# localdevices/pyorc

Measured on AMD Instinct MI355X. Metric: PIV frame-pairs/sec, 1080p 32x32@50% overlap (Mvectors/sec in config), higher is better.
Workload: dtype f32; 1 GPU; synthetic 1080x1920 uint8 particle stack, 1000 frame-pairs per GPU, 32x32 windows @ overlap 16 (BASELINE.json configs[1]); frame_dtype=u8, windows_per_pair=7854, parallelism=single GPU

## Files before the change

pyorc_amd/csrc/fft_debug.hip:

```cpp
#include "piv_fft_impl.h"

namespace lspiv {

template <bool INV, int FORM> __device__ __forceinline__ void fft_form(float (&r)[16], float (&i)[16]) { fft16<INV, false, FORM == 2>(r, i); }
template <bool INV, int FORM> __device__ __forceinline__ void fft_form(float (&r)[32], float (&i)[32]) { fft32<INV, false, FORM == 2>(r, i); }
template <bool INV, int FORM> __device__ __forceinline__ void fft_form(float (&r)[64], float (&i)[64]) { fft64<INV, false, FORM == 2>(r, i); }

template <int N, bool INV, int FORM = 0>
__global__ void fft_debug_kernel(const float* in, float* out, int count) {
  const int t = blockIdx.x * blockDim.x + threadIdx.x;
  if (t >= count) return;
  float r[N], i[N];
#pragma unroll
  for (int j = 0; j < N; ++j) { r[j] = in[(size_t)t * 2 * N + 2 * j]; i[j] = in[(size_t)t * 2 * N + 2 * j + 1]; }
  if constexpr (FORM == 0) fft_n<INV>(r, i); else fft_form<INV, FORM>(r, i);
#pragma unroll
  for (int j = 0; j < N; ++j) { out[(size_t)t * 2 * N + 2 * j] = r[j]; out[(size_t)t * 2 * N + 2 * j + 1] = i[j]; }
}

template <int N, int FORM = 0>
static hipError_t launch_one(bool inverse, const float* in, float* out, int count, hipStream_t s) {
  const dim3 grid((count + 63) / 64), block(64);
  if (inverse) hipLaunchKernelGGL((fft_debug_kernel<N, true, FORM>), grid, block, 0, s, in, out, count);
  else hipLaunchKernelGGL((fft_debug_kernel<N, false, FORM>), grid, block, 0, s, in, out, count);
  return hipGetLastError();
}

hipError_t launch_fft_debug(int n, bool inverse, const float* in, float* out, int count, hipStream_t s) {
  switch (n) {
    case 8: return launch_one<8>(inverse, in, out, count, s);
    case 16: return launch_one<16>(inverse, in, out, count, s);
    case 32: return launch_one<32>(inverse, in, out, count, s);
    case 64: return launch_one<64>(inverse, in, out, count, s);
#define LSPIV_PFA_CASE(m) case m: return launch_one<m>(inverse, in, out, count, s);
    LSPIV_PFA_SIZES(LSPIV_PFA_CASE)
#undef LSPIV_PFA_CASE
    default: return hipErrorInvalidValue;
  }
}

hipError_t launch_fft_debug_form(int n, int form, bool inverse, const float* in, float* out, int count, hipStream_t s) {
  if (form == 0) return launch_fft_debug(n, inverse, in, out, count, s);
  if (form != 1 && form != 2) return hipErrorInvalidValue;
  switch (n) {
    case 16: return form == 1 ? launch_one<16, 1>(inverse, in, out, count, s) : launch_one<16, 2>(inverse, in, out, count, s);
    case 32: return form == 1 ? launch_one<32, 1>(inverse, in, out, count, s) : launch_one<32, 2>(inverse, in, out, count, s);
    case 64: return form == 1 ? launch_one<64, 1>(inverse, in, out, count, s) : launch_one<64, 2>(inverse, in, out, count, s);
    default: return hipErrorInvalidValue;
  }
}

}
```

pyorc_amd/csrc/fft_regs.h:

```cpp
#pragma once
#include <hip/hip_runtime.h>

namespace lspiv {

static constexpr float kCos64[64] = {
    1.0f, 0.9951847195625305f, 0.9807852506637573f, 0.9569403529167175f,
    0.9238795042037964f, 0.8819212913513184f, 0.8314695954322815f, 0.7730104327201843f,
    0.7071067690849304f, 0.6343932747840881f, 0.5555702447891235f, 0.4713967442512512f,
    0.3826834261417389f, 0.290284663438797f, 0.19509032368659973f, 0.0980171412229538f,
    0.0f, -0.0980171412229538f, -0.19509032368659973f, -0.290284663438797f,
    -0.3826834261417389f, -0.4713967442512512f, -0.5555702447891235f, -0.6343932747840881f,
    -0.7071067690849304f, -0.7730104327201843f, -0.8314695954322815f, -0.8819212913513184f,
    -0.9238795042037964f, -0.9569403529167175f, -0.9807852506637573f, -0.9951847195625305f,
    -1.0f, -0.9951847195625305f, -0.9807852506637573f, -0.9569403529167175f,
    -0.9238795042037964f, -0.8819212913513184f, -0.8314695954322815f, -0.7730104327201843f,
    -0.7071067690849304f, -0.6343932747840881f, -0.5555702447891235f, -0.4713967442512512f,
    -0.3826834261417389f, -0.290284663438797f, -0.19509032368659973f, -0.0980171412229538f,
    0.0f, 0.0980171412229538f, 0.19509032368659973f, 0.290284663438797f,
    0.3826834261417389f, 0.4713967442512512f, 0.5555702447891235f, 0.6343932747840881f,
    0.7071067690849304f, 0.7730104327201843f, 0.8314695954322815f, 0.8819212913513184f,
    0.9238795042037964f, 0.9569403529167175f, 0.9807852506637573f, 0.9951847195625305f};

__host__ __device__ constexpr float cos64(int m) { return kCos64[m & 63]; }
__host__ __device__ constexpr float sin64(int m) { return kCos64[(m - 16) & 63]; }

constexpr float kSqrtHalf = 0.70710678118654757f;

template <bool INV, int M>
__device__ __forceinline__ void twiddle64(float& xr, float& xi) {
  constexpr int m = M & 63;
  if constexpr (m == 0) {
    return;
  } else if constexpr (m == 16) {
    float t = xr;
    if constexpr (!INV) { xr = xi; xi = -t; } else { xr = -xi; xi = t; }
  } else if constexpr (m == 32) {
    xr = -xr; xi = -xi;
  } else if constexpr (m == 48) {
    float t = xr;
    if constexpr (!INV) { xr = -xi; xi = t; } else { xr = xi; xi = -t; }
  } else {
    constexpr float c = cos64(m);
    constexpr float s = INV ? sin64(m) : -sin64(m);
    float tr = xr * c - xi * s;
    float ti = xr * s + xi * c;
    xr = tr; xi = ti;
  }
}

template <bool CLAMP>
__device__ __forceinline__ float out01(float x) { return CLAMP ? __builtin_amdgcn_fmed3f(x, 0.0f, 1.0f) : x; }

template <bool INV, bool CLAMP>
__device__ __forceinline__ void bfly4_tail(float ar, float ai, float br, float bi, float cr, float ci, float dr, float di,
                                           float& r0, float& i0, float& r1, float& i1,
                                           float& r2, float& i2, float& r3, float& i3) {
  r0 = out01<CLAMP>(ar + cr); i0 = out01<CLAMP>(ai + ci);
  r2 = out01<CLAMP>(ar - cr); i2 = out01<CLAMP>(ai - ci);
  if constexpr (!INV) {
    r1 = out01<CLAMP>(br + di); i1 = out01<CLAMP>(bi - dr);
    r3 = out01<CLAMP>(br - di); i3 = out01<CLAMP>(bi + dr);
  } else {
    r1 = out01<CLAMP>(br - di); i1 = out01<CLAMP>(bi + dr);
    r3 = out01<CLAMP>(br + di); i3 = out01<CLAMP>(bi - dr);
  }
}

template <bool INV, bool CLAMP = false>
__device__ __forceinline__ void bfly4(float& r0, float& i0, float& r1, float& i1,
                                      float& r2, float& i2, float& r3, float& i3) {
  float ar = r0 + r2, ai = i0 + i2;
  float br = r0 - r2, bi = i0 - i2;
  float cr = r1 + r3, ci = i1 + i3;
  float dr = r1 - r3, di = i1 - i3;
  bfly4_tail<INV, CLAMP>(ar, ai, br, bi, cr, ci, dr, di, r0, i0, r1, i1, r2, i2, r3, i3);
}

template <bool INV, bool CLAMP>
__device__ __forceinline__ void bfly8_tail(float (&r)[8], float (&i)[8]) {
  {
    float tr = r[3], ti = i[3];
    if constexpr (!INV) { r[3] = (tr + ti) * kSqrtHalf; i[3] = (ti - tr) * kSqrtHalf; }
    else                { r[3] = (tr - ti) * kSqrtHalf; i[3] = (ti + tr) * kSqrtHalf; }
    tr = r[5]; ti = i[5];
    if constexpr (!INV) { r[5] = ti; i[5] = -tr; } else { r[5] = -ti; i[5] = tr; }
    tr = r[7]; ti = i[7];
    if constexpr (!INV) { r[7] = (ti - tr) * kSqrtHalf; i[7] = -(tr + ti) * kSqrtHalf; }
    else                { r[7] = -(tr + ti) * kSqrtHalf; i[7] = (tr - ti) * kSqrtHalf; }
  }
  float er[4] = {r[0], r[2], r[4], r[6]}, ei[4] = {i[0], i[2], i[4], i[6]};
  float orr[4] = {r[1], r[3], r[5], r[7]}, oi[4] = {i[1], i[3], i[5], i[7]};
#pragma unroll
  for (int k = 0; k < 4; ++k) {
    r[k] = out01<CLAMP>(er[k] + orr[k]);     i[k] = out01<CLAMP>(ei[k] + oi[k]);
    r[k + 4] = out01<CLAMP>(er[k] - orr[k]); i[k + 4] = out01<CLAMP>(ei[k] - oi[k]);
  }
}

template <bool INV, bool CLAMP = false>
__device__ __forceinline__ void bfly8(float (&r)[8], float (&i)[8]) {
  bfly4<INV>(r[0], i[0], r[2], i[2], r[4], i[4], r[6], i[6]);
  bfly4<INV>(r[1], i[1], r[3], i[3], r[5], i[5], r[7], i[7]);
  bfly8_tail<INV, CLAMP>(r, i);
}

template <bool INV, int N2, int K1, int STEP>
struct TwiddleRow {
  template <int n2>
  static __device__ __forceinline__ void apply(float (&r)[8], float (&i)[8]) {
    if constexpr (n2 < N2) {
      twiddle64<INV, STEP * n2 * K1>(r[n2], i[n2]);
      apply<n2 + 1>(r, i);
    }
  }
};

#ifdef LSPIV_FFT_FOLD
constexpr bool kFftFold16 = LSPIV_FFT_FOLD, kFftFold32 = LSPIV_FFT_FOLD, kFftFold64 = LSPIV_FFT_FOLD, kFftFoldWalk32 = LSPIV_FFT_FOLD;
#else
constexpr bool kFftFold16 = true, kFftFold32 = false, kFftFold64 = false, kFftFoldWalk32 = true;
#endif
template <int N> constexpr bool kFftFoldLen = N == 16 ? kFftFold16 : N == 32 ? kFftFold32 : N == 64 ? kFftFold64 : false;
template <int N> constexpr bool kFftFoldWalk = N == 32 ? kFftFoldWalk32 : kFftFoldLen<N>;

template <bool INV, int M>
struct FoldTw {
  static constexpr int m = M & 63;
  static constexpr bool triv = (m % 16) == 0;
  static constexpr double c = cos64(m), s = INV ? sin64(m) : -sin64(m);
  static constexpr bool sform = (s < 0 ? -s : s) > (c < 0 ? -c : c);
  static constexpr float t = triv ? 0.0f : (float)(sform ? c / s : s / c);
  static constexpr float kr = triv ? 1.0f : (float)(sform ? -s : c);
  static constexpr float ki = triv ? 1.0f : (float)(sform ? s : c);
};

template <bool INV, int M>
__device__ __forceinline__ void fold_u(float& vr, float& vi) {
  using T = FoldTw<INV, M>;
  if constexpr (T::triv) {
    twiddle64<INV, M>(vr, vi);
  } else if constexpr (!T::sform) {
    const float ur = fmaf(vi, -T::t, vr), ui = fmaf(vr, T::t, vi);
    vr = ur; vi = ui;
  } else {
    const float ur = fmaf(vr, -T::t, vi), ui = fmaf(vi, T::t, vr);
    vr = ur; vi = ui;
  }
}

template <bool TRIVX, bool TRIVY>
__device__ __forceinline__ void fold_pair(float x, float kx, float y, float ky, float& sum, float& dif) {
  if constexpr (TRIVX && TRIVY) {
    sum = x + y; dif = x - y;
  } else if constexpr (TRIVY) {
    const float p = kx * x;
    sum = p + y; dif = p - y;
  } else {
    const float p = TRIVX ? x : kx * x;
    sum = fmaf(y, ky, p); dif = fmaf(y, -ky, p);
  }
}

template <bool INV, bool CLAMP, int E0, int E1, int E2, int E3>
__device__ __forceinline__ void bfly4_fold(float& r0, float& i0, float& r1, float& i1,
                                           float& r2, float& i2, float& r3, float& i3) {
  using T0 = FoldTw<INV, E0>; using T1 = FoldTw<INV, E1>; using T2 = FoldTw<INV, E2>; using T3 = FoldTw<INV, E3>;
  fold_u<INV, E0>(r0, i0); fold_u<INV, E1>(r1, i1); fold_u<INV, E2>(r2, i2); fold_u<INV, E3>(r3, i3);
  float ar, ai, br, bi, cr, ci, dr, di;
  fold_pair<T0::triv, T2::triv>(r0, T0::kr, r2, T2::kr, ar, br);
  fold_pair<T0::triv, T2::triv>(i0, T0::ki, i2, T2::ki, ai, bi);
  fold_pair<T1::triv, T3::triv>(r1, T1::kr, r3, T3::kr, cr, dr);
  fold_pair<T1::triv, T3::triv>(i1, T1::ki, i3, T3::ki, ci, di);
  bfly4_tail<INV, CLAMP>(ar, ai, br, bi, cr, ci, dr, di, r0, i0, r1, i1, r2, i2, r3, i3);
}

template <bool INV, bool CLAMP, bool FOLD, int K1, int STEP>
__device__ __forceinline__ void twiddled_bfly8(float (&r)[8], float (&i)[8]) {
  if constexpr (FOLD) {
    constexpr int E = STEP * K1;
    bfly4_fold<INV, false, 0, 2 * E, 4 * E, 6 * E>(r[0], i[0], r[2], i[2], r[4], i[4], r[6], i[6]);
    bfly4_fold<INV, false, E, 3 * E, 5 * E, 7 * E>(r[1], i[1], r[3], i[3], r[5], i[5], r[7], i[7]);
    bfly8_tail<INV, CLAMP>(r, i);
  } else {
    TwiddleRow<INV, 8, K1, STEP>::template apply<1>(r, i);
    bfly8<INV, CLAMP>(r, i);
  }
}

template <bool INV, bool CLAMP, int K1>
__device__ __forceinline__ void fft16_row_fold(const float (&xr)[16], const float (&xi)[16], float (&yr)[16], float (&yi)[16]) {
  float r0 = xr[4 * K1], i0 = xi[4 * K1], r1 = xr[4 * K1 + 1], i1 = xi[4 * K1 + 1];
  float r2 = xr[4 * K1 + 2], i2 = xi[4 * K1 + 2], r3 = xr[4 * K1 + 3], i3 = xi[4 * K1 + 3];
  bfly4_fold<INV, CLAMP, 0, 4 * K1, 8 * K1, 12 * K1>(r0, i0, r1, i1, r2, i2, r3, i3);
  yr[K1] = r0; yi[K1] = i0; yr[K1 + 4] = r1; yi[K1 + 4] = i1; yr[K1 + 8] = r2; yi[K1 + 8] = i2; yr[K1 + 12] = r3; yi[K1 + 12] = i3;
}

template <bool INV, bool CLAMP = false, bool FOLD = kFftFold16>
__device__ __forceinline__ void fft16(float (&xr)[16], float (&xi)[16]) {
#pragma unroll
  for (int n2 = 0; n2 < 4; ++n2)
    bfly4<INV>(xr[n2], xi[n2], xr[4 + n2], xi[4 + n2], xr[8 + n2], xi[8 + n2], xr[12 + n2], xi[12 + n2]);
  if constexpr (FOLD) {
    float yr[16], yi[16];
    fft16_row_fold<INV, CLAMP, 0>(xr, xi, yr, yi); fft16_row_fold<INV, CLAMP, 1>(xr, xi, yr, yi);
    fft16_row_fold<INV, CLAMP, 2>(xr, xi, yr, yi); fft16_row_fold<INV, CLAMP, 3>(xr, xi, yr, yi);
#pragma unroll
    for (int k = 0; k < 16; ++k) { xr[k] = yr[k]; xi[k] = yi[k]; }
    return;
  }
  twiddle64<INV, 4 * 1 * 1>(xr[4 + 1], xi[4 + 1]);  twiddle64<INV, 4 * 2 * 1>(xr[4 + 2], xi[4 + 2]);  twiddle64<INV, 4 * 3 * 1>(xr[4 + 3], xi[4 + 3]);
  twiddle64<INV, 4 * 1 * 2>(xr[8 + 1], xi[8 + 1]);  twiddle64<INV, 4 * 2 * 2>(xr[8 + 2], xi[8 + 2]);  twiddle64<INV, 4 * 3 * 2>(xr[8 + 3], xi[8 + 3]);
  twiddle64<INV, 4 * 1 * 3>(xr[12 + 1], xi[12 + 1]); twiddle64<INV, 4 * 2 * 3>(xr[12 + 2], xi[12 + 2]); twiddle64<INV, 4 * 3 * 3>(xr[12 + 3], xi[12 + 3]);
  float yr[16], yi[16];
#pragma unroll
  for (int k1 = 0; k1 < 4; ++k1) {
    float r0 = xr[4 * k1], i0 = xi[4 * k1], r1 = xr[4 * k1 + 1], i1 = xi[4 * k1 + 1];
    float r2 = xr[4 * k1 + 2], i2 = xi[4 * k1 + 2], r3 = xr[4 * k1 + 3], i3 = xi[4 * k1 + 3];
    bfly4<INV, CLAMP>(r0, i0, r1, i1, r2, i2, r3, i3);
    yr[k1] = r0; yi[k1] = i0; yr[k1 + 4] = r1; yi[k1 + 4] = i1; yr[k1 + 8] = r2; yi[k1 + 8] = i2; yr[k1 + 12] = r3; yi[k1 + 12] = i3;
  }
#pragma unroll
  for (int k = 0; k < 16; ++k) { xr[k] = yr[k]; xi[k] = yi[k]; }
}

template <bool INV, bool CLAMP = false, bool FOLD = kFftFold32>
__device__ __forceinline__ void fft32(float (&xr)[32], float (&xi)[32]) {
#pragma unroll
  for (int n2 = 0; n2 < 8; ++n2)
    bfly4<INV>(xr[n2], xi[n2], xr[8 + n2], xi[8 + n2], xr[16 + n2], xi[16 + n2], xr[24 + n2], xi[24 + n2]);
  float yr[32], yi[32];
  {
    float r[8], i[8];
#pragma unroll
    for (int n2 = 0; n2 < 8; ++n2) { r[n2] = xr[n2]; i[n2] = xi[n2]; }
    bfly8<INV, CLAMP>(r, i);
#pragma unroll
    for (int k2 = 0; k2 < 8; ++k2) { yr[4 * k2] = r[k2]; yi[4 * k2] = i[k2]; }
  }
  {
    float r[8], i[8];
#pragma unroll
    for (int n2 = 0; n2 < 8; ++n2) { r[n2] = xr[8 + n2]; i[n2] = xi[8 + n2]; }
    twiddled_bfly8<INV, CLAMP, FOLD, 1, 2>(r, i);
#pragma unroll
    for (int k2 = 0; k2 < 8; ++k2) { yr[1 + 4 * k2] = r[k2]; yi[1 + 4 * k2] = i[k2]; }
  }
  {
    float r[8], i[8];
#pragma unroll
    for (int n2 = 0; n2 < 8; ++n2) { r[n2] = xr[16 + n2]; i[n2] = xi[16 + n2]; }
    twiddled_bfly8<INV, CLAMP, FOLD, 2, 2>(r, i);
#pragma unroll
    for (int k2 = 0; k2 < 8; ++k2) { yr[2 + 4 * k2] = r[k2]; yi[2 + 4 * k2] = i[k2]; }
  }
  {
    float r[8], i[8];
#pragma unroll
    for (int n2 = 0; n2 < 8; ++n2) { r[n2] = xr[24 + n2]; i[n2] = xi[24 + n2]; }
    twiddled_bfly8<INV, CLAMP, FOLD, 3, 2>(r, i);
#pragma unroll
    for (int k2 = 0; k2 < 8; ++k2) { yr[3 + 4 * k2] = r[k2]; yi[3 + 4 * k2] = i[k2]; }
  }
#pragma unroll
  for (int k = 0; k < 32; ++k) { xr[k] = yr[k]; xi[k] = yi[k]; }
}

template <bool INV, int K1, bool CLAMP = false, bool FOLD = false>
__device__ __forceinline__ void fft64_col(const float (&xr)[64], const float (&xi)[64],
                                          float (&yr)[64], float (&yi)[64]) {
  float r[8], i[8];
#pragma unroll
  for (int n2 = 0; n2 < 8; ++n2) { r[n2] = xr[8 * K1 + n2]; i[n2] = xi[8 * K1 + n2]; }
  twiddled_bfly8<INV, CLAMP, FOLD, K1, 1>(r, i);
#pragma unroll
  for (int k2 = 0; k2 < 8; ++k2) { yr[K1 + 8 * k2] = r[k2]; yi[K1 + 8 * k2] = i[k2]; }
}

#ifndef LSPIV_FFT64_SB
#define LSPIV_FFT64_SB 1
#endif
#ifndef LSPIV_FFT64_PRIO
#define LSPIV_FFT64_PRIO 0
#endif
#define LSPIV_FFT64_BAR do { if (LSPIV_FFT64_SB) __builtin_amdgcn_sched_barrier(0); } while (0)
template <bool INV, bool CLAMP = false, bool FOLD = kFftFold64>
__device__ __forceinline__ void fft64(float (&xr)[64], float (&xi)[64]) {
#pragma unroll
  for (int n2 = 0; n2 < 8; ++n2) {
    float r[8], i[8];
#pragma unroll
    for (int n1 = 0; n1 < 8; ++n1) { r[n1] = xr[8 * n1 + n2]; i[n1] = xi[8 * n1 + n2]; }
    bfly8<INV>(r, i);
#pragma unroll
    for (int k1 = 0; k1 < 8; ++k1) { xr[8 * k1 + n2] = r[k1]; xi[8 * k1 + n2] = i[k1]; }
    if (LSPIV_FFT64_SB) __builtin_amdgcn_sched_barrier(0);
  }
  float yr[64], yi[64];
#if LSPIV_FFT64_PRIO
  __builtin_amdgcn_s_setprio(1);
#endif
  fft64_col<INV, 0, CLAMP, FOLD>(xr, xi, yr, yi); LSPIV_FFT64_BAR;
  fft64_col<INV, 1, CLAMP, FOLD>(xr, xi, yr, yi); LSPIV_FFT64_BAR;
  fft64_col<INV, 2, CLAMP, FOLD>(xr, xi, yr, yi); LSPIV_FFT64_BAR;
  fft64_col<INV, 3, CLAMP, FOLD>(xr, xi, yr, yi); LSPIV_FFT64_BAR;
  fft64_col<INV, 4, CLAMP, FOLD>(xr, xi, yr, yi); LSPIV_FFT64_BAR;
  fft64_col<INV, 5, CLAMP, FOLD>(xr, xi, yr, yi); LSPIV_FFT64_BAR;
  fft64_col<INV, 6, CLAMP, FOLD>(xr, xi, yr, yi); LSPIV_FFT64_BAR;
  fft64_col<INV, 7, CLAMP, FOLD>(xr, xi, yr, yi); LSPIV_FFT64_BAR;
#if LSPIV_FFT64_PRIO
  __builtin_amdgcn_s_setprio(0);
#endif
#pragma unroll
  for (int k = 0; k < 64; ++k) { xr[k] = yr[k]; xi[k] = yi[k]; }
}

template <bool INV>
__device__ __forceinline__ void dft_small(float (&r)[3], float (&i)[3]) {
  constexpr float s3 = 0.86602540378443865f;
  const float tr = r[1] + r[2], ti = i[1] + i[2];
  const float ur = (r[1] - r[2]) * s3, ui = (i[1] - i[2]) * s3;
  const float mr = fmaf(tr, -0.5f, r[0]), mi = fmaf(ti, -0.5f, i[0]);
  r[0] += tr; i[0] += ti;
  if constexpr (!INV) {
    r[1] = mr + ui; i[1] = mi - ur;
    r[2] = mr - ui; i[2] = mi + ur;
  } else {
    r[1] = mr - ui; i[1] = mi + ur;
    r[2] = mr + ui; i[2] = mi - ur;
  }
}
template <bool INV>
__device__ __forceinline__ void dft_small(float (&r)[5], float (&i)[5]) {
// ... 101 lines not shown
      r[k] = mr - vi; i[k] = mi + vr;
      r[P - k] = mr + vi; i[P - k] = mi - vr;
    }
  }
}
template <bool INV> __device__ __forceinline__ void dft_small(float (&r)[7], float (&i)[7]) { dft_odd<INV, 7>(r, i); }
template <bool INV> __device__ __forceinline__ void dft_small(float (&r)[9], float (&i)[9]) { dft_odd<INV, 9>(r, i); }
template <bool INV> __device__ __forceinline__ void dft_small(float (&r)[11], float (&i)[11]) { dft_odd<INV, 11>(r, i); }
template <bool INV> __device__ __forceinline__ void dft_small(float (&r)[13], float (&i)[13]) { dft_odd<INV, 13>(r, i); }
template <bool INV> __device__ __forceinline__ void dft_small(float (&r)[17], float (&i)[17]) { dft_odd<INV, 17>(r, i); }
template <bool INV> __device__ __forceinline__ void dft_small(float (&r)[19], float (&i)[19]) { dft_odd<INV, 19>(r, i); }
template <bool INV> __device__ __forceinline__ void dft_small(float (&r)[23], float (&i)[23]) { dft_odd<INV, 23>(r, i); }
template <bool INV> __device__ __forceinline__ void dft_small(float (&r)[25], float (&i)[25]) { dft_odd<INV, 25>(r, i); }
template <bool INV> __device__ __forceinline__ void dft_small(float (&r)[27], float (&i)[27]) { dft_odd<INV, 27>(r, i); }
template <bool INV> __device__ __forceinline__ void dft_small(float (&r)[29], float (&i)[29]) { dft_odd<INV, 29>(r, i); }
template <bool INV> __device__ __forceinline__ void dft_small(float (&r)[31], float (&i)[31]) { dft_odd<INV, 31>(r, i); }
template <bool INV> __device__ __forceinline__ void fft_pow2(float (&r)[2], float (&i)[2]) {
  const float ar = r[0] + r[1], ai = i[0] + i[1];
  r[1] = r[0] - r[1]; i[1] = i[0] - i[1];
  r[0] = ar; i[0] = ai;
}
template <bool INV> __device__ __forceinline__ void fft_pow2(float (&r)[4], float (&i)[4]) { bfly4<INV>(r[0], i[0], r[1], i[1], r[2], i[2], r[3], i[3]); }
template <bool INV> __device__ __forceinline__ void fft_pow2(float (&r)[8], float (&i)[8]) { bfly8<INV>(r, i); }
template <bool INV> __device__ __forceinline__ void fft_pow2(float (&r)[16], float (&i)[16]) { fft16<INV, false, false>(r, i); }

template <bool INV> __device__ __forceinline__ void fft_pow2(float (&r)[5], float (&i)[5]) { dft_small<INV>(r, i); }
template <bool INV> __device__ __forceinline__ void fft_pow2(float (&r)[7], float (&i)[7]) { dft_small<INV>(r, i); }

template <bool INV> __device__ __forceinline__ void dft_small(float (&r)[15], float (&i)[15]);
template <bool INV> __device__ __forceinline__ void dft_small(float (&r)[21], float (&i)[21]);
constexpr int pfa_unit(int n_self, int n_other) {
  for (int e = n_other; e < n_self * n_other; e += n_other)
    if (e % n_self == 1) return e;
  return 0;
}

template <bool INV, int P, int N2>
__device__ __forceinline__ void fft_pfa(float (&xr)[P * N2], float (&xi)[P * N2]) {
  constexpr int N = P * N2;
  constexpr int e1 = pfa_unit(P, N2), e2 = pfa_unit(N2, P);
  float yr[N], yi[N];
#pragma unroll
  for (int n2 = 0; n2 < N2; ++n2) {
    float r[P], i[P];
#pragma unroll
    for (int n1 = 0; n1 < P; ++n1) { r[n1] = xr[(N2 * n1 + P * n2) % N]; i[n1] = xi[(N2 * n1 + P * n2) % N]; }
    dft_small<INV>(r, i);
// ... 19 lines not shown
```

pyorc_amd/csrc/piv_fft_impl.h:

```cpp
#pragma once
#include <algorithm>
#include <cstdlib>

#include "common.h"
#include "fft_regs.h"

namespace lspiv {

constexpr int WAVES_PER_BLOCK = 4;
constexpr int BLOCK = 64 * WAVES_PER_BLOCK;

template <int N>
struct Geo {
  static constexpr int NN = N * N;
  static constexpr int HALF = N / 2;
  static constexpr bool POW2 = (N & (N - 1)) == 0;
  static constexpr int LG = N <= 16 ? 16 : N <= 32 ? 32 : 64;
  static constexpr bool FULL = N == LG;
  static constexpr int GROUPS = 64 / LG;
  static constexpr int LDS_ROW = N % 4 == 0 ? N + 4 : N + 2;
  static constexpr int LDS_JOB = N * LDS_ROW;
  static constexpr int LDS_BYTES = WAVES_PER_BLOCK * GROUPS * LDS_JOB * 4;
};

// ... 627 lines not shown
template <bool INV> __device__ __forceinline__ void fft_n(float (&xr)[40], float (&xi)[40]) { fft_pfa<INV, 5, 8>(xr, xi); }
template <bool INV> __device__ __forceinline__ void fft_n(float (&xr)[48], float (&xi)[48]) { fft_pfa<INV, 3, 16>(xr, xi); }
template <bool INV> __device__ __forceinline__ void fft_n(float (&xr)[6], float (&xi)[6]) { fft_pfa<INV, 3, 2>(xr, xi); }
template <bool INV> __device__ __forceinline__ void fft_n(float (&xr)[10], float (&xi)[10]) { fft_pfa<INV, 5, 2>(xr, xi); }
template <bool INV> __device__ __forceinline__ void fft_n(float (&xr)[14], float (&xi)[14]) { fft_pfa<INV, 7, 2>(xr, xi); }
template <bool INV> __device__ __forceinline__ void fft_n(float (&xr)[18], float (&xi)[18]) { fft_pfa<INV, 9, 2>(xr, xi); }
template <bool INV> __device__ __forceinline__ void fft_n(float (&xr)[22], float (&xi)[22]) { fft_pfa<INV, 11, 2>(xr, xi); }
template <bool INV> __device__ __forceinline__ void fft_n(float (&xr)[26], float (&xi)[26]) { fft_pfa<INV, 13, 2>(xr, xi); }
template <bool INV> __device__ __forceinline__ void fft_n(float (&xr)[30], float (&xi)[30]) { fft_pfa<INV, 15, 2>(xr, xi); }
template <bool INV> __device__ __forceinline__ void fft_n(float (&xr)[34], float (&xi)[34]) { fft_pfa<INV, 17, 2>(xr, xi); }
template <bool INV> __device__ __forceinline__ void fft_n(float (&xr)[38], float (&xi)[38]) { fft_pfa<INV, 19, 2>(xr, xi); }
template <bool INV> __device__ __forceinline__ void fft_n(float (&xr)[42], float (&xi)[42]) { fft_pfa<INV, 21, 2>(xr, xi); }
template <bool INV> __device__ __forceinline__ void fft_n(float (&xr)[46], float (&xi)[46]) { fft_pfa<INV, 23, 2>(xr, xi); }
template <bool INV> __device__ __forceinline__ void fft_n(float (&xr)[50], float (&xi)[50]) { fft_pfa<INV, 25, 2>(xr, xi); }
template <bool INV> __device__ __forceinline__ void fft_n(float (&xr)[54], float (&xi)[54]) { fft_pfa<INV, 27, 2>(xr, xi); }
template <bool INV> __device__ __forceinline__ void fft_n(float (&xr)[58], float (&xi)[58]) { fft_pfa<INV, 29, 2>(xr, xi); }
template <bool INV> __device__ __forceinline__ void fft_n(float (&xr)[62], float (&xi)[62]) { fft_pfa<INV, 31, 2>(xr, xi); }
template <bool INV> __device__ __forceinline__ void fft_n(float (&xr)[28], float (&xi)[28]) { fft_pfa<INV, 7, 4>(xr, xi); }
template <bool INV> __device__ __forceinline__ void fft_n(float (&xr)[36], float (&xi)[36]) { fft_pfa<INV, 9, 4>(xr, xi); }
template <bool INV> __device__ __forceinline__ void fft_n(float (&xr)[44], float (&xi)[44]) { fft_pfa<INV, 11, 4>(xr, xi); }
template <bool INV> __device__ __forceinline__ void fft_n(float (&xr)[52], float (&xi)[52]) { fft_pfa<INV, 13, 4>(xr, xi); }
template <bool INV> __device__ __forceinline__ void fft_n(float (&xr)[56], float (&xi)[56]) { fft_pfa<INV, 7, 8>(xr, xi); }
template <bool INV> __device__ __forceinline__ void fft_n(float (&xr)[60], float (&xi)[60]) { fft_pfa<INV, 15, 4>(xr, xi); }
template <bool INV, bool CLAMP, bool FOLD, int N>
__device__ __forceinline__ void fft_walk(float (&xr)[N], float (&xi)[N]) {
  static_assert(INV || !CLAMP, "only the inverse transform clips");
  if constexpr (N == 16) fft16<INV, CLAMP, FOLD>(xr, xi);
  else if constexpr (N == 32) fft32<INV, CLAMP, FOLD>(xr, xi);
  else if constexpr (N == 64) fft64<INV, CLAMP, FOLD>(xr, xi);
  else if constexpr (CLAMP) ifft_clamped(xr, xi);
  else fft_n<INV>(xr, xi);
}


template <int N>
__device__ __forceinline__ void cross_spectrum_half(int partner_byte, const float (&zr)[N], const float (&zi)[N],
                                                    float s, float (&rr)[N / 2 + 1], float (&ri)[N / 2 + 1]) {
#pragma unroll
  for (int ky = 0; ky <= N / 2; ++ky) {
    const int kn = (N - ky) % N;
    const float wr = bperm_f(partner_byte, zr[kn]);
    const float wi = bperm_f(partner_byte, zi[kn]);
    const float ar = zr[ky], ai = zi[ky];
    rr[ky] = (2.0f * s) * (ar * wi + ai * wr);
    ri[ky] = s * ((wr * wr + wi * wi) - (ar * ar + ai * ai));
  }
}

template <typename T, int N, bool WANT_NZ, bool EMBED = false, bool SEARCH = false, bool SHIFT = false, bool SHIFT_WIN = false>
__device__ __forceinline__ void correlate_job(const PivParams& p, const TileRef (&t)[2], float* buf, int lg,
                                              int partner_byte, float (&xr)[N], float (&xi)[N], bool (&skip)[2],
                                              float (&mean)[2]) {
// ... 608 lines not shown
    for (int ky = 0; ky <= N / 2; ++ky) fpr[ky] = fpi[ky] = 0.0f;
    prev_dead = true; prev_finite = true; prev_nz = N * N;
  }
};

template <int N>
__device__ __forceinline__ void unpack_step(int ky, float mr, float mi, int partner_byte, WalkCarry<N>& c, float (&xr)[N], float (&xi)[N]) {
  constexpr int H = N / 2;
  const int kn = (N - ky) % N;
  const float pr = xr[ky] + mr, pi = xi[ky] - mi;
  const float ar = c.fpr[ky] * pr + c.fpi[ky] * pi, ai = c.fpr[ky] * pi - c.fpi[ky] * pr;
  c.fpr[ky] = xi[ky] + mi;
  c.fpi[ky] = mr - xr[ky];
  const float qr = c.fpr[ky], qi = c.fpi[ky];
  const float br = pr * qr + pi * qi, bi = pr * qi - pi * qr;
  xr[ky] = ar - bi;
  xi[ky] = ai + br;
  if (ky >= 1 && ky < H) {
    xr[kn] = bperm_f(partner_byte, ar + bi);
    xi[kn] = -bperm_f(partner_byte, ai - br);
  }
}

template <typename T, int N, bool WANT_NZ, bool RELAX = false, bool HALF_TILE = false, int UB = 1, bool U8_EARLY = false, bool FOLD = kFftFoldLen<N>>
__device__ __forceinline__ void walk_iteration(const PivParams& p, const T* row, bool has2, float* buf, int lg,
                                               int partner_byte, int lane0_byte, WalkCarry<N>& c, float (&xr)[N],
                                               float (&xi)[N], float& mean_a, float& mean_b, bool& skip_a, bool& skip_b,
                                               bool& dead_a, bool& dead_b, GlobalF32 acc_slot = nullptr, bool one_job_per_wave_ens = false) {
  using G = Geo<N>;
  constexpr int H = N / 2;
  bool dead0, dead1, fin0 = true, fin1 = true;
  int nz0 = G::NN, nz1 = G::NN;
  if constexpr (LSPIV_PRIO_P != LSPIV_PRIO_E) LSPIV_SETPRIO(LSPIV_PRIO_P);
  if constexpr (sizeof(T) == 4 && kF32Early<N>) {
    const float kHalf = p.std_gain * (1.0f / (2.0f * (float)G::NN));
    const float* r0 = reinterpret_cast<const float*>(row);
    const float* r1 = has2 ? r0 + p.frame_elems : r0;
    load_row_f32<N>(r0, xr);
    load_row_f32<N>(r1, xi);
    const float inv0 = center_clip_f<N, true>(xr, WANT_NZ, p.nz_positive != 0, nz0, fin0);
    const float g0 = inv0 * kHalf;
#pragma unroll
    for (int j = 0; j < N; ++j) xr[j] = __builtin_amdgcn_fmed3f(xr[j] * g0, 0.0f, 1.0f);
    dead0 = inv0 == 0.0f;
    LSPIV_WALK_SB;
    const float inv1 = center_clip_f<N, true>(xi, WANT_NZ, p.nz_positive != 0, nz1, fin1);
    const float g1 = inv1 * kHalf;
// ... 7 lines not shown
      raw1.template fetch<true>(has2 ? row + p.frame_elems : row);
    } else if constexpr (U8_EARLY && sizeof(T) == 1) {
      const T* row1 = has2 ? row + p.frame_elems : row;
      __builtin_amdgcn_sched_barrier(0);
      raw0.fetch(row);
      raw1.fetch(row1);
      __builtin_amdgcn_sched_barrier(0);
    } else {
      raw0.fetch(row);
      raw1.fetch(has2 ? row + p.frame_elems : row);
    }
    prepare_one<T, N, WANT_NZ>(raw0, xr, p.nz_positive != 0, p.std_gain, nz0, fin0, dead0);
    LSPIV_WALK_SB;
    prepare_one<T, N, WANT_NZ>(raw1, xi, p.nz_positive != 0, p.std_gain, nz1, fin1, dead1);
  }
  if constexpr (kEnsLdsRmw<N>) {
    if (one_job_per_wave_ens) {
      dead0 = __builtin_amdgcn_readfirstlane((int)dead0) != 0;
      dead1 = __builtin_amdgcn_readfirstlane((int)dead1) != 0;
    }
  }
  LSPIV_WALK_SB;
  LSPIV_SETPRIO(0);
  fft_walk<false, false, FOLD>(xr, xi);
  LSPIV_WALK_SB;
  LSPIV_SETPRIO(LSPIV_PRIO_T);
  transpose2<N, HALF_TILE>(buf, lg, xr, xi);
  LSPIV_WALK_SB;
  LSPIV_SETPRIO(0);
  fft_walk<false, false, FOLD>(xr, xi);
  LSPIV_WALK_SB;
  LSPIV_SETPRIO(LSPIV_PRIO_U);
  if constexpr (UB <= 1) {
#pragma unroll
    for (int ky = 0; ky <= H; ++ky) {
      const int kn = (N - ky) % N;
      const float mr = bperm_f(partner_byte, xr[kn]);
      const float mi = bperm_f(partner_byte, xi[kn]);
      unpack_step<N>(ky, mr, mi, partner_byte, c, xr, xi);
    }
  } else {
#pragma unroll
    for (int k0 = 0; k0 <= H; k0 += UB) {
      float mr[UB], mi[UB];
#pragma unroll
      for (int b = 0; b < UB && k0 + b <= H; ++b) {
        mr[b] = bperm_f(partner_byte, xr[(N - k0 - b) % N]);
        mi[b] = bperm_f(partner_byte, xi[(N - k0 - b) % N]);
      }
      __builtin_amdgcn_sched_barrier(0);
#pragma unroll
      for (int b = 0; b < UB && k0 + b <= H; ++b) unpack_step<N>(k0 + b, mr[b], mi[b], partner_byte, c, xr, xi);
      __builtin_amdgcn_sched_barrier(0);
    }
  }
  mean_a = bperm_f(lane0_byte, xr[0]);
  mean_b = bperm_f(lane0_byte, xi[0]);
  __builtin_amdgcn_sched_barrier(0);
  LSPIV_SETPRIO(0);
  fft_walk<true, false, FOLD>(xr, xi);
  LSPIV_WALK_SB;
  LSPIV_SETPRIO(LSPIV_PRIO_T);
  transpose2<N, HALF_TILE>(buf, lg, xr, xi);
  if constexpr (kEnsLdsRmw<N>) {
    if (acc_slot) { if constexpr (HALF_TILE) slot_prefetch_lds_upper(acc_slot, buf); else slot_prefetch_lds<N>(acc_slot, buf); }
  }
  LSPIV_WALK_SB;
  LSPIV_SETPRIO(0);
  dead_a = c.prev_dead || dead0;
  dead_b = dead0 || dead1;
  if constexpr (kClampInFft<N>) {
    fft_walk<true, true, FOLD>(xr, xi);
    LSPIV_WALK_SB;
  } else {
    fft_walk<true, false, FOLD>(xr, xi);
    LSPIV_WALK_SB;
    const float hi_a = dead_a ? 0.0f : 1.0f, hi_b = dead_b ? 0.0f : 1.0f;
#pragma unroll
    for (int j = 0; j < N; ++j) {
      xr[j] = __builtin_amdgcn_fmed3f(xr[j], 0.0f, hi_a);
      xi[j] = __builtin_amdgcn_fmed3f(xi[j], 0.0f, hi_b);
    }
  }
  LSPIV_SETPRIO(LSPIV_PRIO_E);
  skip_a = !(c.prev_finite && fin0);
  skip_b = !(fin0 && fin1);
  if (WANT_NZ) {
    skip_a = skip_a || below_threshold<N>(c.prev_nz, nz0, p.signal_threshold);
    skip_b = skip_b || below_threshold<N>(nz0, nz1, p.signal_threshold);
  }
  c.prev_dead = dead1; c.prev_finite = fin1; c.prev_nz = nz1;
}

#ifndef LSPIV_WALK_DEFER
#define LSPIV_WALK_DEFER -1
#endif
constexpr int kDeferSlots = 32, kDeferRecDwords = 8;
constexpr bool kWalkDefer32[3][2][2] = {{{true, true}, {true, true}}, {{true, true}, {true, true}}, {{true, false}, {true, false}}};
// ... 106 lines not shown
  uint32_t it = 0;
  const int partner_byte = partner_byte_of<N>(lane, lg);
  const int lane0_byte = lane0_byte_of<N>();

  const WalkJob wj = walk_job<WAVES_PER_BLOCK * G::GROUPS>((uint32_t)(wave * G::GROUPS + grp), n_seg, p.n_win, p.div_nwin, p.xcd_by_windows);
  const bool job_valid = wj.valid;
  const uint32_t seg = wj.seg;
  const uint32_t win = strip_order(wj.widx, p.strip_w, (uint32_t)p.n_rows, (uint32_t)p.n_cols);
  const uint32_t p0 = seg == 0 ? 0u : p.seg_first + (seg - 1) * seg_len;
  const uint32_t p1 = min(seg == 0 ? p.seg_first : p0 + seg_len, p.n_pairs);
  const uint32_t wrow = p.div_ncols.div(win);
  const uint32_t wcol = win - wrow * (uint32_t)p.n_cols;
  const T* row = static_cast<const T*>(p.frames) + ((int64_t)p0 * p.H + (int64_t)(wrow * p.sy + row_of<N>(lg))) * p.W +
                 (int64_t)wcol * p.sx;
  const float nanv = __builtin_nanf("");

  const bool win_dropped = WANT_NZ && p.win_keep && !p.win_keep[win];
  WalkCarry<N> carry;
  carry.reset();
  for (uint32_t f = p0; f <= p1; f += 2, row += 2 * p.frame_elems) {
    const bool has2 = f + 1 <= p1;
    float xr[N], xi[N], mean_a, mean_b;
    bool skip_a, skip_b, dead_a, dead_b;
    walk_iteration<T, N, WANT_NZ, kWalkRelax<T, N>, false, kWalkUnpackBatch<T, N, PLANES, WANT_NZ>, kWalkU8Early<N, PLANES, WANT_NZ>, kFftFoldWalk<N>>(
        p, row, has2, buf, lg, partner_byte, lane0_byte, carry, xr, xi, mean_a, mean_b, skip_a, skip_b, dead_a, dead_b);
    if (WANT_NZ && win_dropped) skip_a = skip_b = true;
    const bool valid_a = job_valid && f > p0, valid_b = job_valid && has2;
    if constexpr (kTwoPlaneEpilogue<N>) {
      float row_max_a, row_max_b;
      const float vmax_a = plane_max<N>(xr, row_max_a);
      const float vmax_b = plane_max<N>(xi, row_max_b);
      const int ip_a = peak_row<N>(lg, vmax_a, row_max_a);
      const int ip_b = peak_row<N>(lg, vmax_b, row_max_b);
      if (lane_active<N>(lg)) lds_row_write<N>(buf + lg * G::LDS_ROW, xr);
      park_three_rows<N>(mini, lg, xi, ip_b);
      __builtin_amdgcn_wave_barrier();
      const PeakFit<N> fa = peak_fit<N, false>(buf, lg, vmax_a, row_max_a, ip_a, p);
      const PeakFit<N> fb = peak_fit<N, true>(mini, lg, vmax_b, row_max_b, ip_b, p);
      __builtin_amdgcn_wave_barrier();
      const uint32_t g_a = (f - 1) * p.n_win + win, g_b = f * p.n_win + win;
      if (p.rescue_hdr) {
        const bool note_a = valid_a && !dead_a && !skip_a, note_b = valid_b && !dead_b && !skip_b;
        if (note_a) peak_note<N>(buf, lg, fa, p, g_a);
        if (__builtin_amdgcn_ballot_w64(note_b && (fb.pc.amb || fb.pc.fit)) != 0) {
          __builtin_amdgcn_wave_barrier();
          if (lane_active<N>(lg)) lds_row_write<N>(buf + lg * G::LDS_ROW, xi);
          __builtin_amdgcn_wave_barrier();
// ... 771 lines not shown
```

Baseline: 169,900 frame-pairs/s.

## Add split-radix FFT with tangent-factored twiddles for the 32-point walk

Adds a compile-time recursive split-radix FFT that factors each twiddle multiply as a tangent-scaled FMA pair, cutting the real multiply count of the register FFT. It is enabled by default only for the 32-point walk path used in the 32x32 window workload. Other lengths keep the radix-4/8 forms, and a debug form is added. The FFT helpers are also made host-callable for testing. The risks are higher register pressure from the extra temporaries and slightly different rounding.

New measurement: 173,200 frame-pairs/s, median of 6. 1.9% higher.

```diff
diff --git a/pyorc_amd/csrc/fft_debug.hip b/pyorc_amd/csrc/fft_debug.hip
--- a/pyorc_amd/csrc/fft_debug.hip
+++ b/pyorc_amd/csrc/fft_debug.hip
@@ -2,9 +2,9 @@
 
 namespace lspiv {
 
-template <bool INV, int FORM> __device__ __forceinline__ void fft_form(float (&r)[16], float (&i)[16]) { fft16<INV, false, FORM == 2>(r, i); }
-template <bool INV, int FORM> __device__ __forceinline__ void fft_form(float (&r)[32], float (&i)[32]) { fft32<INV, false, FORM == 2>(r, i); }
-template <bool INV, int FORM> __device__ __forceinline__ void fft_form(float (&r)[64], float (&i)[64]) { fft64<INV, false, FORM == 2>(r, i); }
+template <bool INV, int FORM> __device__ __forceinline__ void fft_form(float (&r)[16], float (&i)[16]) { fft16<INV, false, FORM == 2, FORM == 4>(r, i); }
+template <bool INV, int FORM> __device__ __forceinline__ void fft_form(float (&r)[32], float (&i)[32]) { fft32<INV, false, FORM == 2, FORM == 4>(r, i); }
+template <bool INV, int FORM> __device__ __forceinline__ void fft_form(float (&r)[64], float (&i)[64]) { fft64<INV, false, FORM == 2, FORM == 4>(r, i); }
 
 template <int N, bool INV, int FORM = 0>
 __global__ void fft_debug_kernel(const float* in, float* out, int count) {
@@ -41,11 +41,11 @@
 
 hipError_t launch_fft_debug_form(int n, int form, bool inverse, const float* in, float* out, int count, hipStream_t s) {
   if (form == 0) return launch_fft_debug(n, inverse, in, out, count, s);
-  if (form != 1 && form != 2) return hipErrorInvalidValue;
+  if (form != 1 && form != 2 && form != 4) return hipErrorInvalidValue;
   switch (n) {
-    case 16: return form == 1 ? launch_one<16, 1>(inverse, in, out, count, s) : launch_one<16, 2>(inverse, in, out, count, s);
-    case 32: return form == 1 ? launch_one<32, 1>(inverse, in, out, count, s) : launch_one<32, 2>(inverse, in, out, count, s);
-    case 64: return form == 1 ? launch_one<64, 1>(inverse, in, out, count, s) : launch_one<64, 2>(inverse, in, out, count, s);
+    case 16: return form == 1 ? launch_one<16, 1>(inverse, in, out, count, s) : form == 2 ? launch_one<16, 2>(inverse, in, out, count, s) : launch_one<16, 4>(inverse, in, out, count, s);
+    case 32: return form == 1 ? launch_one<32, 1>(inverse, in, out, count, s) : form == 2 ? launch_one<32, 2>(inverse, in, out, count, s) : launch_one<32, 4>(inverse, in, out, count, s);
+    case 64: return form == 1 ? launch_one<64, 1>(inverse, in, out, count, s) : form == 2 ? launch_one<64, 2>(inverse, in, out, count, s) : launch_one<64, 4>(inverse, in, out, count, s);
     default: return hipErrorInvalidValue;
   }
 }
diff --git a/pyorc_amd/csrc/fft_regs.h b/pyorc_amd/csrc/fft_regs.h
--- a/pyorc_amd/csrc/fft_regs.h
+++ b/pyorc_amd/csrc/fft_regs.h
@@ -27,7 +27,7 @@
 constexpr float kSqrtHalf = 0.70710678118654757f;
 
 template <bool INV, int M>
-__device__ __forceinline__ void twiddle64(float& xr, float& xi) {
+__host__ __device__ __forceinline__ void twiddle64(float& xr, float& xi) {
   constexpr int m = M & 63;
   if constexpr (m == 0) {
     return;
@@ -49,10 +49,16 @@
 }
 
 template <bool CLAMP>
-__device__ __forceinline__ float out01(float x) { return CLAMP ? __builtin_amdgcn_fmed3f(x, 0.0f, 1.0f) : x; }
+__host__ __device__ __forceinline__ float out01(float x) {
+#if defined(__HIP_DEVICE_COMPILE__)
+  return CLAMP ? __builtin_amdgcn_fmed3f(x, 0.0f, 1.0f) : x;
+#else
+  return CLAMP ? (x < 0.0f ? 0.0f : x > 1.0f ? 1.0f : x) : x;
+#endif
+}
 
 template <bool INV, bool CLAMP>
-__device__ __forceinline__ void bfly4_tail(float ar, float ai, float br, float bi, float cr, float ci, float dr, float di,
+__host__ __device__ __forceinline__ void bfly4_tail(float ar, float ai, float br, float bi, float cr, float ci, float dr, float di,
                                            float& r0, float& i0, float& r1, float& i1,
                                            float& r2, float& i2, float& r3, float& i3) {
   r0 = out01<CLAMP>(ar + cr); i0 = out01<CLAMP>(ai + ci);
@@ -67,7 +73,7 @@
 }
 
 template <bool INV, bool CLAMP = false>
-__device__ __forceinline__ void bfly4(float& r0, float& i0, float& r1, float& i1,
+__host__ __device__ __forceinline__ void bfly4(float& r0, float& i0, float& r1, float& i1,
                                       float& r2, float& i2, float& r3, float& i3) {
   float ar = r0 + r2, ai = i0 + i2;
   float br = r0 - r2, bi = i0 - i2;
@@ -77,7 +83,7 @@
 }
 
 template <bool INV, bool CLAMP>
-__device__ __forceinline__ void bfly8_tail(float (&r)[8], float (&i)[8]) {
+__host__ __device__ __forceinline__ void bfly8_tail(float (&r)[8], float (&i)[8]) {
   {
     float tr = r[3], ti = i[3];
     if constexpr (!INV) { r[3] = (tr + ti) * kSqrtHalf; i[3] = (ti - tr) * kSqrtHalf; }
@@ -98,7 +104,7 @@
 }
 
 template <bool INV, bool CLAMP = false>
-__device__ __forceinline__ void bfly8(float (&r)[8], float (&i)[8]) {
+__host__ __device__ __forceinline__ void bfly8(float (&r)[8], float (&i)[8]) {
   bfly4<INV>(r[0], i[0], r[2], i[2], r[4], i[4], r[6], i[6]);
   bfly4<INV>(r[1], i[1], r[3], i[3], r[5], i[5], r[7], i[7]);
   bfly8_tail<INV, CLAMP>(r, i);
@@ -107,7 +113,7 @@
 template <bool INV, int N2, int K1, int STEP>
 struct TwiddleRow {
   template <int n2>
-  static __device__ __forceinline__ void apply(float (&r)[8], float (&i)[8]) {
+  static __host__ __device__ __forceinline__ void apply(float (&r)[8], float (&i)[8]) {
     if constexpr (n2 < N2) {
       twiddle64<INV, STEP * n2 * K1>(r[n2], i[n2]);
       apply<n2 + 1>(r, i);
@@ -135,7 +141,7 @@
 };
 
 template <bool INV, int M>
-__device__ __forceinline__ void fold_u(float& vr, float& vi) {
+__host__ __device__ __forceinline__ void fold_u(float& vr, float& vi) {
   using T = FoldTw<INV, M>;
   if constexpr (T::triv) {
     twiddle64<INV, M>(vr, vi);
@@ -149,7 +155,7 @@
 }
 
 template <bool TRIVX, bool TRIVY>
-__device__ __forceinline__ void fold_pair(float x, float kx, float y, float ky, float& sum, float& dif) {
+__host__ __device__ __forceinline__ void fold_pair(float x, float kx, float y, float ky, float& sum, float& dif) {
   if constexpr (TRIVX && TRIVY) {
     sum = x + y; dif = x - y;
   } else if constexpr (TRIVY) {
@@ -162,7 +168,7 @@
 }
 
 template <bool INV, bool CLAMP, int E0, int E1, int E2, int E3>
-__device__ __forceinline__ void bfly4_fold(float& r0, float& i0, float& r1, float& i1,
+__host__ __device__ __forceinline__ void bfly4_fold(float& r0, float& i0, float& r1, float& i1,
                                            float& r2, float& i2, float& r3, float& i3) {
   using T0 = FoldTw<INV, E0>; using T1 = FoldTw<INV, E1>; using T2 = FoldTw<INV, E2>; using T3 = FoldTw<INV, E3>;
   fold_u<INV, E0>(r0, i0); fold_u<INV, E1>(r1, i1); fold_u<INV, E2>(r2, i2); fold_u<INV, E3>(r3, i3);
@@ -175,7 +181,7 @@
 }
 
 template <bool INV, bool CLAMP, bool FOLD, int K1, int STEP>
-__device__ __forceinline__ void twiddled_bfly8(float (&r)[8], float (&i)[8]) {
+__host__ __device__ __forceinline__ void twiddled_bfly8(float (&r)[8], float (&i)[8]) {
   if constexpr (FOLD) {
     constexpr int E = STEP * K1;
     bfly4_fold<INV, false, 0, 2 * E, 4 * E, 6 * E>(r[0], i[0], r[2], i[2], r[4], i[4], r[6], i[6]);
@@ -187,16 +193,91 @@
   }
 }
 
+#ifdef LSPIV_FFT_SR
+constexpr bool kFftSr16 = LSPIV_FFT_SR, kFftSr32 = LSPIV_FFT_SR, kFftSr64 = LSPIV_FFT_SR, kFftSrWalk32 = LSPIV_FFT_SR;
+#else
+constexpr bool kFftSr16 = false, kFftSr32 = false, kFftSr64 = false, kFftSrWalk32 = true;
+#endif
+template <int N> constexpr bool kFftSrLen = N == 16 ? kFftSr16 : N == 32 ? kFftSr32 : N == 64 ? kFftSr64 : false;
+template <int N> constexpr bool kFftSrWalk = N == 32 ? kFftSrWalk32 : kFftSrLen<N>;
+
+template <int N, int NT, int OFF, int STRIDE, bool CLAMP>
+__host__ __device__ __forceinline__ void sr_fft(const float (&xr)[NT], const float (&xi)[NT], float (&yr)[N], float (&yi)[N]);
+
+template <int N, int K, bool CLAMP>
+__host__ __device__ __forceinline__ void sr_step(const float (&er)[N / 2], const float (&ei)[N / 2], const float (&zr)[N / 4], const float (&zi)[N / 4],
+                                                 const float (&wr)[N / 4], const float (&wi)[N / 4], float (&yr)[N], float (&yi)[N]) {
+  constexpr int Q = N / 4, m = K * (64 / N);
+  if constexpr (K == 0) {
+    const float sr = zr[0] + wr[0], si = zi[0] + wi[0], dr = zr[0] - wr[0], di = zi[0] - wi[0];
+    yr[0] = out01<CLAMP>(er[0] + sr);         yi[0] = out01<CLAMP>(ei[0] + si);
+    yr[2 * Q] = out01<CLAMP>(er[0] - sr);     yi[2 * Q] = out01<CLAMP>(ei[0] - si);
+    yr[Q] = out01<CLAMP>(er[Q] + di);         yi[Q] = out01<CLAMP>(ei[Q] - dr);
+    yr[3 * Q] = out01<CLAMP>(er[Q] - di);     yi[3 * Q] = out01<CLAMP>(ei[Q] + dr);
+  } else {
+    constexpr double c = cos64(m), s = sin64(m);
+    if constexpr (s <= c) {
+      constexpr float t = (float)(s / c), k = (float)c;
+      const float ur = fmaf(zi[K], t, zr[K]), ui = fmaf(zr[K], -t, zi[K]);
+      const float vr = fmaf(wi[K], -t, wr[K]), vi = fmaf(wr[K], t, wi[K]);
+      const float sr = ur + vr, si = ui + vi, dr = ur - vr, di = ui - vi;
+      yr[K] = out01<CLAMP>(fmaf(sr, k, er[K]));              yi[K] = out01<CLAMP>(fmaf(si, k, ei[K]));
+      yr[K + 2 * Q] = out01<CLAMP>(fmaf(sr, -k, er[K]));     yi[K + 2 * Q] = out01<CLAMP>(fmaf(si, -k, ei[K]));
+      yr[K + Q] = out01<CLAMP>(fmaf(di, k, er[K + Q]));      yi[K + Q] = out01<CLAMP>(fmaf(dr, -k, ei[K + Q]));
+      yr[K + 3 * Q] = out01<CLAMP>(fmaf(di, -k, er[K + Q])); yi[K + 3 * Q] = out01<CLAMP>(fmaf(dr, k, ei[K + Q]));
+    } else {
+      constexpr float t = (float)(c / s), k = (float)s;
+      const float ur = fmaf(zr[K], t, zi[K]), ui = fmaf(zi[K], -t, zr[K]);
+      const float vr = fmaf(wr[K], -t, wi[K]), vi = fmaf(wi[K], t, wr[K]);
+      const float sr = ur - vr, si = vi - ui, dr = ur + vr, dn = ui + vi;
+      yr[K] = out01<CLAMP>(fmaf(sr, k, er[K]));              yi[K] = out01<CLAMP>(fmaf(si, k, ei[K]));
+      yr[K + 2 * Q] = out01<CLAMP>(fmaf(sr, -k, er[K]));     yi[K + 2 * Q] = out01<CLAMP>(fmaf(si, -k, ei[K]));
+      yr[K + Q] = out01<CLAMP>(fmaf(dn, -k, er[K + Q]));     yi[K + Q] = out01<CLAMP>(fmaf(dr, -k, ei[K + Q]));
+      yr[K + 3 * Q] = out01<CLAMP>(fmaf(dn, k, er[K + Q]));  yi[K + 3 * Q] = out01<CLAMP>(fmaf(dr, k, ei[K + Q]));
+    }
+  }
+  if constexpr (K + 1 < Q) sr_step<N, K + 1, CLAMP>(er, ei, zr, zi, wr, wi, yr, yi);
+}
+
+template <int N, int NT, int OFF, int STRIDE, bool CLAMP>
+__host__ __device__ __forceinline__ void sr_fft(const float (&xr)[NT], const float (&xi)[NT], float (&yr)[N], float (&yi)[N]) {
+  static_assert(N * STRIDE == NT && (N & (N - 1)) == 0 && N <= 64, "a power of two, and the strides of its own recursion");
+  constexpr int o0 = OFF & (NT - 1);
+  if constexpr (N == 1) {
+    yr[0] = out01<CLAMP>(xr[o0]); yi[0] = out01<CLAMP>(xi[o0]);
+  } else if constexpr (N == 2) {
+    constexpr int o1 = (OFF + STRIDE) & (NT - 1);
+    yr[0] = out01<CLAMP>(xr[o0] + xr[o1]); yi[0] = out01<CLAMP>(xi[o0] + xi[o1]);
+    yr[1] = out01<CLAMP>(xr[o0] - xr[o1]); yi[1] = out01<CLAMP>(xi[o0] - xi[o1]);
+  } else {
+    float er[N / 2], ei[N / 2], zr[N / 4], zi[N / 4], wr[N / 4], wi[N / 4];
+    sr_fft<N / 2, NT, OFF, 2 * STRIDE, false>(xr, xi, er, ei);
+    sr_fft<N / 4, NT, OFF + STRIDE, 4 * STRIDE, false>(xr, xi, zr, zi);
+    sr_fft<N / 4, NT, OFF - STRIDE + NT, 4 * STRIDE, false>(xr, xi, wr, wi);
+    sr_step<N, 0, CLAMP>(er, ei, zr, zi, wr, wi, yr, yi);
+  }
+}
+
+template <bool INV, bool CLAMP, int N>
+__host__ __device__ __forceinline__ void fft_sr(float (&xr)[N], float (&xi)[N]) {
+  float yr[N], yi[N];
+  if constexpr (INV) sr_fft<N, N, 0, 1, CLAMP>(xi, xr, yi, yr);
+  else sr_fft<N, N, 0, 1, CLAMP>(xr, xi, yr, yi);
+#pragma unroll
+  for (int k = 0; k < N; ++k) { xr[k] = yr[k]; xi[k] = yi[k]; }
+}
+
 template <bool INV, bool CLAMP, int K1>
-__device__ __forceinline__ void fft16_row_fold(const float (&xr)[16], const float (&xi)[16], float (&yr)[16], float (&yi)[16]) {
+__host__ __device__ __forceinline__ void fft16_row_fold(const float (&xr)[16], const float (&xi)[16], float (&yr)[16], float (&yi)[16]) {
   float r0 = xr[4 * K1], i0 = xi[4 * K1], r1 = xr[4 * K1 + 1], i1 = xi[4 * K1 + 1];
   float r2 = xr[4 * K1 + 2], i2 = xi[4 * K1 + 2], r3 = xr[4 * K1 + 3], i3 = xi[4 * K1 + 3];
   bfly4_fold<INV, CLAMP, 0, 4 * K1, 8 * K1, 12 * K1>(r0, i0, r1, i1, r2, i2, r3, i3);
   yr[K1] = r0; yi[K1] = i0; yr[K1 + 4] = r1; yi[K1 + 4] = i1; yr[K1 + 8] = r2; yi[K1 + 8] = i2; yr[K1 + 12] = r3; yi[K1 + 12] = i3;
 }
 
-template <bool INV, bool CLAMP = false, bool FOLD = kFftFold16>
-__device__ __forceinline__ void fft16(float (&xr)[16], float (&xi)[16]) {
+template <bool INV, bool CLAMP = false, bool FOLD = kFftFold16, bool SR = kFftSr16>
+__host__ __device__ __forceinline__ void fft16(float (&xr)[16], float (&xi)[16]) {
+  if constexpr (SR) { fft_sr<INV, CLAMP>(xr, xi); return; }
 #pragma unroll
   for (int n2 = 0; n2 < 4; ++n2)
     bfly4<INV>(xr[n2], xi[n2], xr[4 + n2], xi[4 + n2], xr[8 + n2], xi[8 + n2], xr[12 + n2], xi[12 + n2]);
@@ -223,8 +304,9 @@
   for (int k = 0; k < 16; ++k) { xr[k] = yr[k]; xi[k] = yi[k]; }
 }
 
-template <bool INV, bool CLAMP = false, bool FOLD = kFftFold32>
-__device__ __forceinline__ void fft32(float (&xr)[32], float (&xi)[32]) {
+template <bool INV, bool CLAMP = false, bool FOLD = kFftFold32, bool SR = kFftSr32>
+__host__ __device__ __forceinline__ void fft32(float (&xr)[32], float (&xi)[32]) {
+  if constexpr (SR) { fft_sr<INV, CLAMP>(xr, xi); return; }
 #pragma unroll
   for (int n2 = 0; n2 < 8; ++n2)
     bfly4<INV>(xr[n2], xi[n2], xr[8 + n2], xi[8 + n2], xr[16 + n2], xi[16 + n2], xr[24 + n2], xi[24 + n2]);
@@ -266,7 +348,7 @@
 }
 
 template <bool INV, int K1, bool CLAMP = false, bool FOLD = false>
-__device__ __forceinline__ void fft64_col(const float (&xr)[64], const float (&xi)[64],
+__host__ __device__ __forceinline__ void fft64_col(const float (&xr)[64], const float (&xi)[64],
                                           float (&yr)[64], float (&yi)[64]) {
   float r[8], i[8];
 #pragma unroll
@@ -282,9 +364,14 @@
 #ifndef LSPIV_FFT64_PRIO
 #define LSPIV_FFT64_PRIO 0
 #endif
+#if defined(__HIP_DEVICE_COMPILE__)
 #define LSPIV_FFT64_BAR do { if (LSPIV_FFT64_SB) __builtin_amdgcn_sched_barrier(0); } while (0)
-template <bool INV, bool CLAMP = false, bool FOLD = kFftFold64>
-__device__ __forceinline__ void fft64(float (&xr)[64], float (&xi)[64]) {
+#else
+#define LSPIV_FFT64_BAR do { } while (0)
+#endif
+template <bool INV, bool CLAMP = false, bool FOLD = kFftFold64, bool SR = kFftSr64>
+__host__ __device__ __forceinline__ void fft64(float (&xr)[64], float (&xi)[64]) {
+  if constexpr (SR) { fft_sr<INV, CLAMP>(xr, xi); return; }
 #pragma unroll
   for (int n2 = 0; n2 < 8; ++n2) {
     float r[8], i[8];
@@ -293,10 +380,10 @@
     bfly8<INV>(r, i);
 #pragma unroll
     for (int k1 = 0; k1 < 8; ++k1) { xr[8 * k1 + n2] = r[k1]; xi[8 * k1 + n2] = i[k1]; }
-    if (LSPIV_FFT64_SB) __builtin_amdgcn_sched_barrier(0);
+    LSPIV_FFT64_BAR;
   }
   float yr[64], yi[64];
-#if LSPIV_FFT64_PRIO
+#if LSPIV_FFT64_PRIO && defined(__HIP_DEVICE_COMPILE__)
   __builtin_amdgcn_s_setprio(1);
 #endif
   fft64_col<INV, 0, CLAMP, FOLD>(xr, xi, yr, yi); LSPIV_FFT64_BAR;
@@ -307,7 +394,7 @@
   fft64_col<INV, 5, CLAMP, FOLD>(xr, xi, yr, yi); LSPIV_FFT64_BAR;
   fft64_col<INV, 6, CLAMP, FOLD>(xr, xi, yr, yi); LSPIV_FFT64_BAR;
   fft64_col<INV, 7, CLAMP, FOLD>(xr, xi, yr, yi); LSPIV_FFT64_BAR;
-#if LSPIV_FFT64_PRIO
+#if LSPIV_FFT64_PRIO && defined(__HIP_DEVICE_COMPILE__)
   __builtin_amdgcn_s_setprio(0);
 #endif
 #pragma unroll
@@ -455,7 +542,7 @@
 }
 template <bool INV> __device__ __forceinline__ void fft_pow2(float (&r)[4], float (&i)[4]) { bfly4<INV>(r[0], i[0], r[1], i[1], r[2], i[2], r[3], i[3]); }
 template <bool INV> __device__ __forceinline__ void fft_pow2(float (&r)[8], float (&i)[8]) { bfly8<INV>(r, i); }
-template <bool INV> __device__ __forceinline__ void fft_pow2(float (&r)[16], float (&i)[16]) { fft16<INV, false, false>(r, i); }
+template <bool INV> __device__ __forceinline__ void fft_pow2(float (&r)[16], float (&i)[16]) { fft16<INV, false, false, false>(r, i); }
 
 template <bool INV> __device__ __forceinline__ void fft_pow2(float (&r)[5], float (&i)[5]) { dft_small<INV>(r, i); }
 template <bool INV> __device__ __forceinline__ void fft_pow2(float (&r)[7], float (&i)[7]) { dft_small<INV>(r, i); }
diff --git a/pyorc_amd/csrc/piv_fft_impl.h b/pyorc_amd/csrc/piv_fft_impl.h
--- a/pyorc_amd/csrc/piv_fft_impl.h
+++ b/pyorc_amd/csrc/piv_fft_impl.h
@@ -673,12 +673,12 @@
 template <bool INV> __device__ __forceinline__ void fft_n(float (&xr)[52], float (&xi)[52]) { fft_pfa<INV, 13, 4>(xr, xi); }
 template <bool INV> __device__ __forceinline__ void fft_n(float (&xr)[56], float (&xi)[56]) { fft_pfa<INV, 7, 8>(xr, xi); }
 template <bool INV> __device__ __forceinline__ void fft_n(float (&xr)[60], float (&xi)[60]) { fft_pfa<INV, 15, 4>(xr, xi); }
-template <bool INV, bool CLAMP, bool FOLD, int N>
+template <bool INV, bool CLAMP, bool FOLD, bool SR, int N>
 __device__ __forceinline__ void fft_walk(float (&xr)[N], float (&xi)[N]) {
   static_assert(INV || !CLAMP, "only the inverse transform clips");
-  if constexpr (N == 16) fft16<INV, CLAMP, FOLD>(xr, xi);
-  else if constexpr (N == 32) fft32<INV, CLAMP, FOLD>(xr, xi);
-  else if constexpr (N == 64) fft64<INV, CLAMP, FOLD>(xr, xi);
+  if constexpr (N == 16) fft16<INV, CLAMP, FOLD, SR>(xr, xi);
+  else if constexpr (N == 32) fft32<INV, CLAMP, FOLD, SR>(xr, xi);
+  else if constexpr (N == 64) fft64<INV, CLAMP, FOLD, SR>(xr, xi);
   else if constexpr (CLAMP) ifft_clamped(xr, xi);
   else fft_n<INV>(xr, xi);
 }
@@ -1333,7 +1333,7 @@
   }
 }
 
-template <typename T, int N, bool WANT_NZ, bool RELAX = false, bool HALF_TILE = false, int UB = 1, bool U8_EARLY = false, bool FOLD = kFftFoldLen<N>>
+template <typename T, int N, bool WANT_NZ, bool RELAX = false, bool HALF_TILE = false, int UB = 1, bool U8_EARLY = false, bool FOLD = kFftFoldLen<N>, bool SR = kFftSrLen<N>>
 __device__ __forceinline__ void walk_iteration(const PivParams& p, const T* row, bool has2, float* buf, int lg,
                                                int partner_byte, int lane0_byte, WalkCarry<N>& c, float (&xr)[N],
                                                float (&xi)[N], float& mean_a, float& mean_b, bool& skip_a, bool& skip_b,
@@ -1387,13 +1387,13 @@
   }
   LSPIV_WALK_SB;
   LSPIV_SETPRIO(0);
-  fft_walk<false, false, FOLD>(xr, xi);
+  fft_walk<false, false, FOLD, SR>(xr, xi);
   LSPIV_WALK_SB;
   LSPIV_SETPRIO(LSPIV_PRIO_T);
   transpose2<N, HALF_TILE>(buf, lg, xr, xi);
   LSPIV_WALK_SB;
   LSPIV_SETPRIO(0);
-  fft_walk<false, false, FOLD>(xr, xi);
+  fft_walk<false, false, FOLD, SR>(xr, xi);
   LSPIV_WALK_SB;
   LSPIV_SETPRIO(LSPIV_PRIO_U);
   if constexpr (UB <= 1) {
@@ -1423,7 +1423,7 @@
   mean_b = bperm_f(lane0_byte, xi[0]);
   __builtin_amdgcn_sched_barrier(0);
   LSPIV_SETPRIO(0);
-  fft_walk<true, false, FOLD>(xr, xi);
+  fft_walk<true, false, FOLD, SR>(xr, xi);
   LSPIV_WALK_SB;
   LSPIV_SETPRIO(LSPIV_PRIO_T);
   transpose2<N, HALF_TILE>(buf, lg, xr, xi);
@@ -1435,10 +1435,10 @@
   dead_a = c.prev_dead || dead0;
   dead_b = dead0 || dead1;
   if constexpr (kClampInFft<N>) {
-    fft_walk<true, true, FOLD>(xr, xi);
+    fft_walk<true, true, FOLD, SR>(xr, xi);
     LSPIV_WALK_SB;
   } else {
-    fft_walk<true, false, FOLD>(xr, xi);
+    fft_walk<true, false, FOLD, SR>(xr, xi);
     LSPIV_WALK_SB;
     const float hi_a = dead_a ? 0.0f : 1.0f, hi_b = dead_b ? 0.0f : 1.0f;
 #pragma unroll
@@ -1591,7 +1591,7 @@
     const bool has2 = f + 1 <= p1;
     float xr[N], xi[N], mean_a, mean_b;
     bool skip_a, skip_b, dead_a, dead_b;
-    walk_iteration<T, N, WANT_NZ, kWalkRelax<T, N>, false, kWalkUnpackBatch<T, N, PLANES, WANT_NZ>, kWalkU8Early<N, PLANES, WANT_NZ>, kFftFoldWalk<N>>(
+    walk_iteration<T, N, WANT_NZ, kWalkRelax<T, N>, false, kWalkUnpackBatch<T, N, PLANES, WANT_NZ>, kWalkU8Early<N, PLANES, WANT_NZ>, kFftFoldWalk<N>, kFftSrWalk<N>>(
         p, row, has2, buf, lg, partner_byte, lane0_byte, carry, xr, xi, mean_a, mean_b, skip_a, skip_b, dead_a, dead_b);
     if (WANT_NZ && win_dropped) skip_a = skip_b = true;
     const bool valid_a = job_valid && f > p0, valid_b = job_valid && has2;
```
